# leaner-forever/SEGS-SLAM

Hardware: AMD Instinct MI355X
Metric: mapper train-iters/sec (fwd+bwd raster) (higher is better)
Workload: dtype f32; 1 GPU; 1080p_3m: 3000000 Gaussians, 1920x1080, 1 keyframe per GPU, fwd+bwd raster; P=3000000, P_visible=2096178, num_rendered=10472370, instances_binned=7913347, instances_live=6766534, width=1920, height=1080, parallelism=keyframe-dp1, forward=resident (no host sync), hipgraph=off

## Files before the change

include/segs_raster.h:

```cpp
#ifndef SEGS_RASTER_H_
#define SEGS_RASTER_H_

#include <stddef.h>
#include <stdint.h>

#ifdef __cplusplus
extern "C" {
#endif

#define SEGS_OK 0
#define SEGS_ERR_INVALID_ARGUMENT (-1)
#define SEGS_ERR_UNSUPPORTED (-2)
#define SEGS_ERR_ALLOC (-3)

typedef char* (*segs_alloc_fn)(void* ctx, size_t bytes);

const char* segs_last_error(void);

#define SEGS_RASTER_SKIP_NONPOSITIVE_OPACITY 1u
#define SEGS_RASTER_KEEP_DEAD_INSTANCES 2u
#define SEGS_RASTER_GATHER_TILES_TOUCHED 4u
#define SEGS_RASTER_TEST_NARROW_PACK 8u
#define SEGS_RASTER_UNFUSED_BINNING 16u
#define SEGS_RASTER_TIGHT_BINNING 32u
#define SEGS_RASTER_MFMA_MOMENTS 64u
uint32_t segs_raster_set_flags(uint32_t flags);

uint32_t* segs_raster_set_status_mirror(uint32_t* host_mapped_status);

size_t segs_geometry_bytes(int P);
size_t segs_image_bytes(int width, int height);
size_t segs_binning_bytes(int num_rendered);

int segs_rasterize_forward(segs_alloc_fn geometry_alloc, void* geometry_ctx,
                           segs_alloc_fn binning_alloc, void* binning_ctx,
                           segs_alloc_fn image_alloc, void* image_ctx,
                           int P, int D, int M,
                           const float* background, int width, int height,
                           const float* means3D, const float* shs, const float* colors_precomp,
                           const float* opacities, const float* scales, float scale_modifier,
// ... 28 lines not shown
int segs_project2_image(int P, int D, int M, int width, int height, const float* means3D, const float* shs,
                        const float* colors_precomp, const float* opacities, const float* scales,
                        float scale_modifier, const float* rotations, const float* cov3D_precomp,
                        const float* viewmatrix, const float* projmatrix, const float* cam_pos,
                        float tan_fovx, float tan_fovy, int prefiltered, float* out_color, float* points_image,
                        int* radii, void* stream);

int segs_debug_unpack_geometry(const char* geom_buffer, int P, const int* radii, float* means2D ,
                               float* conic_opacity , float* depths , uint32_t* tiles_touched ,
                               uint32_t* point_offsets , float* rgb , void* stream);
int segs_debug_unpack_binning(const char* binning_buffer, const char* geom_buffer, int P, int R, int width, int height,
                              uint64_t* keys_sorted , uint32_t* point_list , void* stream);
int segs_debug_instance_values(const char* binning_buffer, int R, uint32_t* values , void* stream);
int segs_debug_unpack_image(const char* image_buffer, int width, int height, uint32_t* ranges ,
                            float* final_T , uint32_t* n_contrib , void* stream);

int segs_debug_preprocess_backward(int P, int width, int height, const float* means3D, const int* radii,
                                   const float* scales, float scale_modifier, const float* rotations,
                                   const float* cov3D_precomp, const float* viewmatrix, const float* projmatrix,
                                   float tan_fovx, float tan_fovy, const float* dL_dmean2D, const float* dL_dconic,
                                   float* dL_dmean3D, float* dL_dcov3D, float* dL_dscale, float* dL_drot, void* stream);

int segs_sort_pairs(const uint64_t* keys_in, const uint32_t* vals_in, uint64_t* keys_out, uint32_t* vals_out,
                    int n, int end_bit, char* temp, void* stream);

size_t segs_resident_binning_bytes(int P, int capacity);
int segs_rasterize_forward_resident(char* geom_buffer, char* binning_buffer, char* image_buffer, int capacity,
                                    int geom_rows, int P, int D, int M, const float* background, int width, int height,
                                    const float* means3D, const float* shs, const float* colors_precomp,
                                    const float* opacities, const float* scales, float scale_modifier,
// ... 124 lines not shown
```

segs-slam_amd/_capi.py:

```python
from __future__ import annotations

import ctypes as C
import os
import subprocess

_HERE = os.path.dirname(os.path.abspath(__file__))
CSRC = os.path.join(_HERE, "csrc")
LIB_PATH = os.environ.get("SEGS_RASTER_LIB") or os.path.join(CSRC, "libsegs_raster.so")

ALLOC_FN = C.CFUNCTYPE(C.c_void_p, C.c_void_p, C.c_size_t)


class NeuralDims(C.Structure):
    _fields_ = [("feat_dim", C.c_int), ("n_offsets", C.c_int), ("appearance_dim", C.c_int), ("use_feat_bank", C.c_int),
                ("add_opacity_dist", C.c_int), ("add_cov_dist", C.c_int), ("add_color_dist", C.c_int)]


class ProjectionTargets(C.Structure):
    _fields_ = [("records", C.c_void_p), ("radii", C.c_void_p), ("tiles_touched", C.c_void_p), ("depth_keys", C.c_void_p),
                ("tile_ranges", C.c_void_p), ("depth_overflow", C.c_void_p), ("num_tiles", C.c_int), ("flags", C.c_uint32)]


class DepthOutputs(C.Structure):
    _fields_ = [("depth", C.c_void_p), ("alpha", C.c_void_p)]
# ... 31 lines not shown
    "segs_raster_set_status_mirror": (_vp, [_vp]),
    "segs_training_statis": (_i, [_i, _i] + [_vp] * 9),
    "segs_training_statis_guarded": (_i, [_i, _i] + [_vp] * 10),
    "segs_anchor_growing_temp_bytes": (_sz, [_i, _i]),
    "segs_anchor_growing_level": (_i, [_i, _i, _i, _i] + [_vp] * 7 + [_f, _f, _f, _i] + [_vp] * 5),
    "segs_depth_seed_temp_bytes": (_sz, [_i, _i, _i, _i]),
    "segs_depth_seed": (_i, [_i, _vp, _i, _i, _vp, _vp, _vp, _f, _f, _vp, _vp, _i, _vp, _vp, _vp, _vp, _vp]),
    "segs_neural_set_flags": (C.c_uint, [C.c_uint]),
    "segs_neural_param_layout": (_i, [_vp, _vp, _vp, _vp, _vp]),
    "segs_neural_temp_bytes": (_sz, [_vp, _i]),
    "segs_neural_forward": (_i, [_vp, _i] + [_vp] * 16),
    "segs_neural_forward_projected": (_i, [_vp, _i] + [_vp] * 16 + [_i, _i, _f, _f, _f, _vp, _vp]),
    "segs_neural_backward": (_i, [_vp, _i] + [_vp] * 17 + [_f, _vp, _vp, _vp]),
    "segs_neural_backward_camera": (_i, [_vp, _i] + [_vp] * 17 + [_f, _vp, _vp, _vp, _vp]),
    "segs_geometry_bytes": (_sz, [_i]),
    "segs_image_bytes": (_sz, [_i, _i]),
    "segs_binning_bytes": (_sz, [_i]),
    "segs_rasterize_forward": (_i, [ALLOC_FN, _vp, ALLOC_FN, _vp, ALLOC_FN, _vp, _i, _i, _i, _vp, _i, _i, _vp, _vp, _vp,
                                     _vp, _vp, _f, _vp, _vp, _vp, _vp, _vp, _f, _f, _i, _vp, _vp, _vp, C.POINTER(_i)]),
    "segs_rasterize_backward": (_i, [_i, _i, _i, _i, _vp, _i, _i, _vp, _vp, _vp, _vp, _f, _vp, _vp, _vp, _vp, _vp, _f, _f,
                                      _vp, _vp, _vp, _vp, _vp, _vp, _vp, _vp, _vp, _vp, _vp, _vp, _vp, _vp, _vp]),
    "segs_resident_binning_bytes": (_sz, [_i, _i]),
    "segs_rasterize_forward_resident": (_i, [_vp, _vp, _vp, _i, _i, _i, _i, _i, _vp, _i, _i, _vp, _vp, _vp, _vp, _vp, _f, _vp, _vp, _vp,
                                              _vp, _vp, _f, _f, _vp, _vp, _vp, _vp]),
    "segs_resident_projection_targets": (_i, [_vp, _vp, _vp, _i, _i, _i, _i, _i, _vp, _vp, _vp]),
    "segs_rasterize_forward_resident_projected": (_i, [_vp, _vp, _vp, _i, _i, _i, _vp, _i, _i, _vp, _vp, _vp]),
    "segs_rasterize_backward_resident": (_i, [_vp, _vp, _vp, _i, _i, _i, _i, _i, _vp, _i, _i, _vp, _vp, _vp, _f, _vp, _vp, _vp, _vp, _vp,
                                               _f, _f, _vp, _vp, _vp, _vp, _vp, _vp, _vp, _vp, _vp, _vp, _vp, _vp]),
}
for _name in ("segs_rasterize_forward", "segs_rasterize_backward", "segs_rasterize_forward_resident",
# ... 117 lines not shown
```

segs-slam_amd/csrc/capi.hip:

```cpp
#include <hip/hip_runtime.h>
#include <cstdio>
#include <cstdlib>
#include <algorithm>
#include <cstring>
#include <string>
#include <vector>
#include "../../include/segs_raster.h"
#include "gs_layout.h"
#include "kernels.h"

using namespace segs;

namespace {
thread_local std::string g_err;
}
int segs::set_error(int code, const char* what) {
  g_err = what;
  return code;
}
int segs::set_hip_error(hipError_t e, const char* where) {
  g_err = std::string(where) + ": " + hipGetErrorString(e);
  return (int)e > 0 ? (int)e : 1;
}

// ... 130 lines not shown
  return SEGS_OK;
}

struct Geom {
  GeomLayout L;
  char* base;
  float* rec() const { return (float*)(base + L.rec); }
  BinInfo* bin() const { return (BinInfo*)(base + L.bin); }
  uint32_t* offsets() const { return (uint32_t*)(base + L.offsets); }
  int* radii_internal() const { return (int*)(base + L.radii_internal); }
  uint32_t* block_sums() const { return (uint32_t*)(base + L.block_sums); }
  uint32_t* num_rendered() const { return (uint32_t*)(base + L.num_rendered); }
  uint32_t* clamped() const { return (uint32_t*)(base + L.clamped); }
  float* gacc() const { return (float*)(base + L.gacc); }
  uint32_t* touched() const { return (uint32_t*)(base + L.touched); }
};
Geom geom_at(char* p, int P) { return Geom{geom_layout(P), align_ptr(p)}; }
Geom geom_at(char* p, int P, int rows) {
  Geom g{geom_layout(rows), align_ptr(p)};
  g.L.P = P;
  g.L.nblocks = (P + 255) / 256;
  return g;
}

int run_preprocess(const Geom& G, int P, int W, int H, const float* means3D, const float* colors, const float* opac,
                   const float* scales, float mod, const float* rots, const float* cov3D_precomp, const float* view,
                   const float* proj, float tan_fovx, float tan_fovy, int* radii, const float* shs, int D, int M,
                   const float* cam_pos, hipStream_t st, uint32_t* depth_keys = nullptr, uint32_t* depth_vals = nullptr,
                   uint2* ranges = nullptr, uint32_t extra_flags = 0u, uint32_t* depth_overflow = nullptr) {
  const float focal_y = H / (2.0f * tan_fovy);
// ... 122 lines not shown

uint32_t* segs_raster_set_status_mirror(uint32_t* host_mapped_status) {
  uint32_t* old = g_status_mirror;
  g_status_mirror = host_mapped_status;
  return old;
}

uint32_t segs_raster_set_flags(uint32_t flags) {
  const uint32_t old = g_flags;
  g_flags = flags;
  return old;
}

size_t segs_geometry_bytes(int P) { return geom_layout(P < 0 ? 0 : P).total; }
size_t segs_image_bytes(int width, int height) { return image_layout(width, height).total; }
size_t segs_binning_bytes(int num_rendered) { return binning_layout(num_rendered < 0 ? 0 : num_rendered).total; }

static int rasterize_forward_impl(segs_alloc_fn geometry_alloc, void* geometry_ctx, segs_alloc_fn binning_alloc, void* binning_ctx,
                           segs_alloc_fn image_alloc, void* image_ctx, int P, int D, int M, const float* background,
                           int width, int height, const float* means3D, const float* shs, const float* colors_precomp,
                           const float* opacities, const float* scales, float scale_modifier, const float* rotations,
                           const float* cov3D_precomp, const float* viewmatrix, const float* projmatrix,
                           const float* cam_pos, float tan_fovx, float tan_fovy, int prefiltered, float* out_color,
                           int* radii, const segs_depth_outputs* dout, void* stream, int* num_rendered) {
  (void)prefiltered;
  hipStream_t st = (hipStream_t)stream;
  if (!geometry_alloc || !binning_alloc || !image_alloc) return fail(SEGS_ERR_INVALID_ARGUMENT, "null allocator callback");
  if (P < 0 || width <= 0 || height <= 0) return fail(SEGS_ERR_INVALID_ARGUMENT, "bad P / image size");
  if (P > MAX_GAUSSIANS) return fail(SEGS_ERR_INVALID_ARGUMENT, "P exceeds 2^28 Gaussians (sort values carry a 4-bit quadrant mask)");
  if (!background || !out_color || !viewmatrix || !projmatrix || !num_rendered) return fail(SEGS_ERR_INVALID_ARGUMENT, "null required pointer");
// ... 121 lines not shown
  Geom G = geom_at(geom_buffer, P, geom_rows);
  if (!radii) radii = G.radii_internal();
  const ImageLayout IL = image_layout(width, height);
  const BinningLayout BL = binning_layout(R);
  char* img = align_ptr(image_buffer);
  char* bin = align_ptr(binning_buffer);
  const uint32_t gx = (width + TILE_X - 1) / TILE_X, gy = (height + TILE_Y - 1) / TILE_Y;
  const float focal_y = height / (2.0f * tan_fovy), focal_x = width / (2.0f * tan_fovx);

  if (!self_clean) { PROF(K_MEMSET);
  HIP_TRY(hipMemsetAsync(G.gacc(), 0, (size_t)P * GACC_DWORDS * 4, st));
  }
  const float* dL_ddepth = dgrad ? dgrad->dL_ddepth : nullptr;
  const float* dL_dalpha = dgrad ? dgrad->dL_dalpha : nullptr;
  const bool depth_form = dL_ddepth || dL_dalpha;
  if (R > 0 && depth_form) {
    { PROF(K_RENDER_BWD);
    render_bwd_depth_kernel<<<(gx * gy + 7) / 8 * 32, 64, 0, st>>>((const uint2*)(img + IL.ranges), (const uint32_t*)(bin + BL.vals[0]), width,
                                                                  height, G.rec(), background, (const float*)(img + IL.final_T),
                                                                  (const uint32_t*)(img + IL.n_contrib), dL_dpix, G.gacc(), gx * gy,
                                                                  dL_ddepth, dL_dalpha);
    }
    LAUNCH_TRY("render_bwd_depth_kernel");
  } else if (R > 0) {
    { PROF(K_RENDER_BWD);
    static const bool mfma_env = [] { const char* e = getenv("SEGS_RENDER_BWD_MFMA"); return e && e[0] == '1'; }();
    ((mfma_env || (g_flags & SEGS_RASTER_MFMA_MOMENTS)) ? render_bwd_mfma_kernel : render_bwd_kernel)<<<(gx * gy + 7) / 8 * 32, 64, 0, st>>>((const uint2*)(img + IL.ranges), (const uint32_t*)(bin + BL.vals[0]), width,
                                                    height, G.rec(), background, (const float*)(img + IL.final_T),
                                                    (const uint32_t*)(img + IL.n_contrib), dL_dpix, G.gacc(), gx * gy);
    }
    LAUNCH_TRY("render_bwd_kernel");
  }
  { PROF(K_PREPROCESS_BWD);
  auto* const kernel = cam_live ? (dL_ddepth ? preprocess_bwd_kernel<true, true> : preprocess_bwd_kernel<false, true>)
                                : (dL_ddepth ? preprocess_bwd_kernel<true, false> : preprocess_bwd_kernel<false, false>);
  kernel<<<G.L.nblocks, 256, 0, st>>>(P, means3D, radii, cov3D_precomp ? nullptr : scales, rotations,
                                                     scale_modifier, cov3D_precomp, viewmatrix, projmatrix, focal_x, focal_y,
                                                     tan_fovx, tan_fovy, G.gacc(), (float)width, (float)height, dL_dmean2D, dL_dconic, dL_dopacity, dL_dcolor,
                                                     dL_dmean3D, dL_dcov3D, dL_dscale, dL_drot, self_clean ? 1 : 0, nullptr,
                                                     cam_live ? camera_partials(cam) : nullptr);
  LAUNCH_TRY("preprocess_bwd_kernel");
  if (cam_live)
    if (int rc = camera_grads_finish(cam, G.L.nblocks, st)) return rc;
  }
  if (shs) {
    sh_backward_kernel<<<G.L.nblocks, 256, 0, st>>>(P, means3D, radii, shs, D, M, campos, G.clamped(), dL_dcolor, dL_dmean3D, dL_dsh);
    LAUNCH_TRY("sh_backward_kernel");
  }
  return SEGS_OK;
}

int segs_rasterize_backward(int P, int D, int M, int R, const float* background, int width, int height,
                            const float* means3D, const float* shs, const float* colors_precomp, const float* scales,
                            float scale_modifier, const float* rotations, const float* cov3D_precomp,
                            const float* viewmatrix, const float* projmatrix, const float* campos, float tan_fovx,
// ... 151 lines not shown

int segs_debug_preprocess_backward(int P, int width, int height, const float* means3D, const int* radii, const float* scales,
                                   float scale_modifier, const float* rotations, const float* cov3D_precomp,
                                   const float* viewmatrix, const float* projmatrix, float tan_fovx, float tan_fovy,
                                   const float* dL_dmean2D, const float* dL_dconic, float* dL_dmean3D, float* dL_dcov3D,
                                   float* dL_dscale, float* dL_drot, void* stream) {
  hipStream_t st = (hipStream_t)stream;
  if (P <= 0) return SEGS_OK;
  if (!means3D || !radii || !viewmatrix || !projmatrix || !dL_dmean2D || !dL_dconic || !dL_dmean3D || !dL_dcov3D)
    return fail(SEGS_ERR_INVALID_ARGUMENT, "null pointer");
  const float focal_y = height / (2.0f * tan_fovy), focal_x = width / (2.0f * tan_fovx);
  preprocess_bwd_kernel<false, false><<<(P + 255) / 256, 256, 0, st>>>(P, means3D, radii, cov3D_precomp ? nullptr : scales, rotations,
                                                         scale_modifier, cov3D_precomp, viewmatrix, projmatrix, focal_x, focal_y,
                                                         tan_fovx, tan_fovy, nullptr, (float)width, (float)height, const_cast<float*>(dL_dmean2D),
                                                         const_cast<float*>(dL_dconic), nullptr, nullptr, dL_dmean3D, dL_dcov3D,
                                                         dL_dscale, dL_drot, 0, nullptr, nullptr);
  LAUNCH_TRY("preprocess_bwd_kernel");
  return SEGS_OK;
}

int segs_debug_preprocess_backward_camera(int P, int width, int height, const float* means3D, const int* radii, const float* scales,
                                          float scale_modifier, const float* rotations, const float* cov3D_precomp,
                                          const float* viewmatrix, const float* projmatrix, float tan_fovx, float tan_fovy,
                                          const float* dL_dmean2D, const float* dL_dconic, float* dL_dmean3D, float* dL_dcov3D,
                                          float* dL_dscale, float* dL_drot, const float* dL_dz, const segs_camera_grads* camera_grads,
                                          void* stream) {
  if (!camera_grads)
    return segs_debug_preprocess_backward(P, width, height, means3D, radii, scales, scale_modifier, rotations, cov3D_precomp, viewmatrix,
                                          projmatrix, tan_fovx, tan_fovy, dL_dmean2D, dL_dconic, dL_dmean3D, dL_dcov3D, dL_dscale, dL_drot,
                                          stream);
  hipStream_t st = (hipStream_t)stream;
  bool cam_live = false;
  if (int rc = camera_grads_begin(camera_grads, nullptr, P <= 0, st, &cam_live)) return rc;
  if (P <= 0) return SEGS_OK;
  if (!means3D || !radii || !viewmatrix || !projmatrix || !dL_dmean2D || !dL_dconic || !dL_dmean3D || !dL_dcov3D)
    return fail(SEGS_ERR_INVALID_ARGUMENT, "null pointer");
  const float focal_y = height / (2.0f * tan_fovy), focal_x = width / (2.0f * tan_fovx);
  const int nblocks = (P + 255) / 256;
  (dL_dz ? preprocess_bwd_kernel<true, true> : preprocess_bwd_kernel<false, true>)<<<nblocks, 256, 0, st>>>(
      P, means3D, radii, cov3D_precomp ? nullptr : scales, rotations, scale_modifier, cov3D_precomp, viewmatrix, projmatrix, focal_x,
      focal_y, tan_fovx, tan_fovy, nullptr, (float)width, (float)height, const_cast<float*>(dL_dmean2D), const_cast<float*>(dL_dconic),
      nullptr, nullptr, dL_dmean3D, dL_dcov3D, dL_dscale, dL_drot, 0, dL_dz, camera_partials(camera_grads));
  LAUNCH_TRY("preprocess_bwd_kernel");
  return camera_grads_finish(camera_grads, nblocks, st);
}

int segs_sort_pairs(const uint64_t* keys_in, const uint32_t* vals_in, uint64_t* keys_out, uint32_t* vals_out, int n,
                    int end_bit, char* temp, void* stream) {
  hipStream_t st = (hipStream_t)stream;
  if (n < 0 || end_bit <= 0 || end_bit > 64) return fail(SEGS_ERR_INVALID_ARGUMENT, "bad n / end_bit");
  if (n == 0) return SEGS_OK;
  if (!keys_in || !vals_in || !keys_out || !vals_out || !temp) return fail(SEGS_ERR_INVALID_ARGUMENT, "null pointer");
  const BinningLayout BL = binning_layout(n);
  char* bin = align_ptr(temp);
  const int passes = (end_bit + 7) / 8;
  const int side = passes & 1;
  HIP_TRY(hipMemcpyAsync(bin + BL.keys[side], keys_in, (size_t)n * 8, hipMemcpyDeviceToDevice, st));
// ... 235 lines not shown
```

segs-slam_amd/csrc/gs_layout.h:

```cpp
#pragma once
#include <algorithm>
#include <cstddef>
#include <cstdint>

namespace segs {

constexpr int TILE_X = 16;
constexpr int TILE_Y = 16;
constexpr int NUM_CHANNELS = 3;

constexpr float LOG2E = 1.4426950408889634f;

constexpr int REC_DWORDS = 16;
enum RecField { REC_X = 0, REC_Y, REC_A2, REC_B2, REC_C2, REC_O, REC_R, REC_G, REC_B, REC_DEPTH, REC_RECT_MIN, REC_RECT_MAX, REC_CA, REC_CB, REC_CC };

struct BinInfo { uint32_t depth_bits, rect_min, rect_max, tiles_touched; };
constexpr uint32_t ID_BITS = 28;
constexpr uint32_t ID_MASK = (1u << ID_BITS) - 1u;
constexpr int MAX_GAUSSIANS = 1 << ID_BITS;

constexpr int GACC_DWORDS = 16;

constexpr size_t ALIGN = 256;
inline size_t align_up(size_t v, size_t a = ALIGN) { return (v + a - 1) / a * a; }

struct GeomLayout {
  size_t rec, bin, offsets, radii_internal, block_sums, clamped, num_rendered, gacc, touched, total;
  int P, nblocks;
};
inline GeomLayout geom_layout(int P) {
  GeomLayout g{};
  g.P = P;
  g.nblocks = (P + 255) / 256;
  size_t o = 0;
  g.rec = o;            o = align_up(o + (size_t)P * REC_DWORDS * 4);
  g.bin = o;            o = align_up(o + (size_t)P * sizeof(BinInfo));
  g.offsets = o;        o = align_up(o + (size_t)P * 4);
  g.radii_internal = o; o = align_up(o + (size_t)P * 4);
  g.block_sums = o;     o = align_up(o + (size_t)(g.nblocks + 1) * 4 * 3);
  g.clamped = o;        o = align_up(o + (size_t)P * 4);
  g.num_rendered = o;   o = align_up(o + 64);
  g.gacc = o;           o = align_up(o + (size_t)P * GACC_DWORDS * 4);
  g.touched = o;        o = align_up(o + (size_t)P * 4);
  g.total = o + ALIGN;
  return g;
}

struct ImageLayout {
  size_t ranges, final_T, n_contrib, total;
};
inline ImageLayout image_layout(int W, int H) {
  ImageLayout l{};
  const size_t tiles = (size_t)((W + TILE_X - 1) / TILE_X) * ((H + TILE_Y - 1) / TILE_Y);
  size_t o = 0;
  l.ranges = o;    o = align_up(o + tiles * 8);
  l.final_T = o;   o = align_up(o + (size_t)W * H * 4);
  l.n_contrib = o; o = align_up(o + (size_t)W * H * 4);
  l.total = o + ALIGN;
// ... 58 lines not shown
```

segs-slam_amd/csrc/kernels.h:

```cpp
#pragma once
#include <hip/hip_runtime.h>
#include <cstdint>
#include "gs_layout.h"

namespace segs {

int set_error(int code, const char* what);
int set_hip_error(hipError_t e, const char* where);


__global__ void preprocess_fwd_kernel(
    int P, const float* __restrict__ means3D, const float* __restrict__ scales, float mod,
    const float* __restrict__ rotations, const float* __restrict__ opacities, const float* __restrict__ colors,
    const float* __restrict__ cov3D_precomp, const float* __restrict__ viewmatrix, const float* __restrict__ projmatrix,
    int W, int H, float tan_fovx, float tan_fovy, float focal_x, float focal_y, uint32_t gx, uint32_t gy,
    int* __restrict__ radii, float* __restrict__ rec, BinInfo* __restrict__ bin, uint32_t* __restrict__ block_sums,
    uint32_t* __restrict__ depth_range, const float* __restrict__ shs, int D, int M, const float* __restrict__ cam_pos,
    uint32_t* __restrict__ clamped, uint32_t flags, uint32_t* __restrict__ depth_keys, uint32_t* __restrict__ depth_vals,
    uint2* __restrict__ ranges, int num_tiles, uint32_t* __restrict__ depth_overflow, uint32_t* __restrict__ touched_dense);
constexpr uint32_t DEPTH_KEY_MIN = 0x3E4CCCCDu;
constexpr int DEPTH_KEY_BITS = 27;

__global__ void visible_filter_kernel(
    int P, const float* __restrict__ means3D, const float* __restrict__ scales, float mod,
// ... 3 lines not shown
    int log_scale_stride);

__global__ void mark_visible_kernel(int P, const float* __restrict__ means3D, const float* __restrict__ viewmatrix,
                                    uint8_t* __restrict__ present);

constexpr int CAM_SUMS = 24;
template <bool DEPTH, bool CAM>
__global__ void preprocess_bwd_kernel(
    int P, const float* __restrict__ means3D, const int* __restrict__ radii, const float* __restrict__ scales,
    const float* __restrict__ rotations, float mod, const float* __restrict__ cov3D_precomp,
    const float* __restrict__ view, const float* __restrict__ proj, float h_x, float h_y, float tan_fovx, float tan_fovy,
    float* __restrict__ gacc, float img_w, float img_h,
    float* __restrict__ dL_dmean2D, float* __restrict__ dL_dconic,
    float* __restrict__ dL_dopacity, float* __restrict__ dL_dcolor, float* __restrict__ dL_dmean3D,
    float* __restrict__ dL_dcov3D, float* __restrict__ dL_dscale, float* __restrict__ dL_drot, int clean_gacc,
    const float* __restrict__ dz_in, float* __restrict__ cam_partials);
__global__ void camera_grad_reduce_kernel(const float* __restrict__ partials, int nblocks, float* __restrict__ dL_dview,
                                          float* __restrict__ dL_dproj);
__global__ void sh_backward_kernel(int P, const float* __restrict__ means3D, const int* __restrict__ radii,
                                   const float* __restrict__ shs, int D, int M, const float* __restrict__ cam_pos,
                                   const uint32_t* __restrict__ clamped, const float* __restrict__ dL_dcolor,
                                   float* __restrict__ dL_dmean3D, float* __restrict__ dL_dsh);

__global__ void scan_block_sums_kernel(uint32_t* __restrict__ block_sums, int nblocks, const uint32_t* __restrict__ depth_range,
                                       uint32_t* __restrict__ total);
__global__ void ordered_offsets_kernel(int P, const uint32_t* __restrict__ block_sums, uint32_t* __restrict__ incl,
                                       uint32_t* __restrict__ total_out, const uint32_t* __restrict__ ng_dev,
                                       uint32_t* __restrict__ first_owner, uint32_t owner_entries);
__global__ void duplicate_with_keys_kernel(int P, int R, const float* __restrict__ rec,
                                           const uint32_t* __restrict__ order, const uint32_t* __restrict__ incl,
                                           uint32_t* __restrict__ keys, uint32_t* __restrict__ vals, uint32_t gx,
// ... 15 lines not shown
                                     const uint32_t* __restrict__ digit_totals, int nblocks, int nchunks,
                                     const uint32_t* __restrict__ n_dev, int drop_dead, uint32_t* __restrict__ n_live_out,
                                     const uint32_t* __restrict__ aux_in, uint32_t* __restrict__ aux_out, int nbits, int chunk_tiles, int pack_shift,
                                     uint2* __restrict__ ranges_out, uint32_t* __restrict__ status, uint32_t* __restrict__ status_mirror,
                                     int write_keys);
__global__ void identify_tile_ranges_kernel(int L, const uint32_t* __restrict__ keys, uint2* __restrict__ ranges,
                                            const uint32_t* __restrict__ n_dev, uint32_t* __restrict__ status,
                                            uint32_t* __restrict__ status_mirror, const uint32_t* __restrict__ n_live);

__global__ void render_fwd_kernel(const uint2* __restrict__ ranges, const uint32_t* __restrict__ point_list, int W, int H,
                                  const float* __restrict__ rec, const float* __restrict__ bg,
                                  float* __restrict__ final_T, uint32_t* __restrict__ n_contrib, float* __restrict__ out_color);
__global__ void render_bwd_kernel(const uint2* __restrict__ ranges, const uint32_t* __restrict__ point_list, int W, int H,
                                  const float* __restrict__ rec, const float* __restrict__ bg,
                                  const float* __restrict__ final_T, const uint32_t* __restrict__ n_contrib,
                                  const float* __restrict__ dL_dpix, float* __restrict__ gacc, uint32_t num_tiles);
__global__ void render_bwd_mfma_kernel(const uint2* __restrict__ ranges, const uint32_t* __restrict__ point_list, int W, int H,
                                       const float* __restrict__ rec, const float* __restrict__ bg,
                                       const float* __restrict__ final_T, const uint32_t* __restrict__ n_contrib,
                                       const float* __restrict__ dL_dpix, float* __restrict__ gacc, uint32_t num_tiles);
__global__ void render_fwd_depth_kernel(const uint2* __restrict__ ranges, const uint32_t* __restrict__ point_list, int W, int H,
                                        const float* __restrict__ rec, const float* __restrict__ bg,
                                        float* __restrict__ final_T, uint32_t* __restrict__ n_contrib, float* __restrict__ out_color,
                                        float* __restrict__ out_depth, float* __restrict__ out_alpha);
__global__ void render_bwd_depth_kernel(const uint2* __restrict__ ranges, const uint32_t* __restrict__ point_list, int W, int H,
                                        const float* __restrict__ rec, const float* __restrict__ bg,
                                        const float* __restrict__ final_T, const uint32_t* __restrict__ n_contrib,
                                        const float* __restrict__ dL_dpix, float* __restrict__ gacc, uint32_t num_tiles,
                                        const float* __restrict__ dL_ddepth, const float* __restrict__ dL_dalpha);

__global__ void unpack_geometry_kernel(int P, const float* __restrict__ rec, const BinInfo* __restrict__ bin,
                                       const int* __restrict__ radii, float* __restrict__ means2D,
                                       float* __restrict__ conic_opacity, float* __restrict__ depths,
                                       uint32_t* __restrict__ tiles_touched, float* __restrict__ rgb);

__global__ void rebuild_keys_kernel(int R, const uint32_t* __restrict__ tile_keys, const uint32_t* __restrict__ vals,
                                    const BinInfo* __restrict__ bin, uint64_t* __restrict__ keys64);
__global__ void make_depth_keys_kernel(int P, const BinInfo* __restrict__ bin, uint32_t dcull, uint32_t* __restrict__ keys,
                                       uint32_t* __restrict__ vals, uint2* __restrict__ ranges, int num_tiles);
__global__ void ordered_block_sums_kernel(int P, const uint32_t* touched, const uint32_t* __restrict__ order,
                                          uint32_t* __restrict__ block_sums, uint32_t* sorted_touched,
                                          const uint32_t* __restrict__ ng_dev, uint32_t* __restrict__ order_rw, int pack_shift);
__global__ void point_offsets_kernel(int P, const BinInfo* __restrict__ bin, uint32_t* __restrict__ offsets);
__global__ void strip_mask_kernel(int n, const uint32_t* __restrict__ vals, uint32_t* __restrict__ out);
// ... 3 lines not shown
```

segs-slam_amd/csrc/preprocess.hip:

```cpp
#include <hip/hip_runtime.h>
#include <cstdint>
#include "gs_layout.h"
#include "kernels.h"
#include "project_gaussian.h"
#include "sh_color.h"

#pragma clang fp contract(off)

namespace segs {

__device__ __forceinline__ float3 load_row3(const float* __restrict__ a, int P, float* lds ) {
  const int tid = threadIdx.x;
  const size_t base = (size_t)blockIdx.x * 768;
  const size_t lim = (size_t)P * 3;
#pragma unroll
  for (int k = 0; k < 3; k++) {
    const size_t i = base + k * 256 + tid;
    lds[k * 256 + tid] = i < lim ? a[i] : 0.f;
  }
  __syncthreads();
  float3 v = make_float3(lds[3 * tid], lds[3 * tid + 1], lds[3 * tid + 2]);
  __syncthreads();
  return v;
}
// ... 178 lines not shown
  R[0][0] = 1.f - 2.f * (y * y + z * z); R[0][1] = 2.f * (x * y - r * z);       R[0][2] = 2.f * (x * z + r * y);
  R[1][0] = 2.f * (x * y + r * z);       R[1][1] = 1.f - 2.f * (x * x + z * z); R[1][2] = 2.f * (y * z - r * x);
  R[2][0] = 2.f * (x * z - r * y);       R[2][1] = 2.f * (y * z + r * x);       R[2][2] = 1.f - 2.f * (x * x + y * y);
}

template <bool DEPTH, bool CAM>
__global__ void __launch_bounds__(256) preprocess_bwd_kernel(
    int P, const float* __restrict__ means3D, const int* __restrict__ radii, const float* __restrict__ scales,
    const float* __restrict__ rotations, float mod, const float* __restrict__ cov3D_precomp,
    const float* __restrict__ view, const float* __restrict__ proj, float h_x, float h_y, float tan_fovx, float tan_fovy,
    float* __restrict__ gacc, float img_w, float img_h,
    float* __restrict__ dL_dmean2D, float* __restrict__ dL_dconic,
    float* __restrict__ dL_dopacity, float* __restrict__ dL_dcolor, float* __restrict__ dL_dmean3D,
    float* __restrict__ dL_dcov3D, float* __restrict__ dL_dscale, float* __restrict__ dL_drot,
    int clean_gacc ,
    const float* __restrict__ dz_in, float* __restrict__ cam_partials ) {
  __shared__ float lds[3 * 768];
  const int idx = blockIdx.x * 256 + threadIdx.x;
  const bool live = idx < P;
  const bool binned = live && radii[idx] > 0;
  float3 mean, scale, unused;
  load_rows3(means3D, scales, nullptr, P, lds, mean, scale, unused);

  float g2x = 0.f, g2y = 0.f;
  Sym2 G{0.f, 0.f, 0.f};
  float dcol0 = 0.f, dcol1 = 0.f, dcol2 = 0.f, dop = 0.f, dz = 0.f;
  float4 a0 = make_float4(0.f, 0.f, 0.f, 0.f), a1 = a0;
  if (gacc) {
    {
      __shared__ __attribute__((aligned(16))) float gl[4][32 * GACC_DWORDS];
      const int lane = threadIdx.x & 63;
      float* const wl = gl[threadIdx.x >> 6];
      const uint64_t rows = __ballot(binned);
      const size_t wave_first = (size_t)blockIdx.x * 256 + (threadIdx.x & ~63);
#pragma unroll
      for (int half = 0; half < 2; half++) {
        float4 q[2];
#pragma unroll
        for (int j = 0; j < 2; j++) {
          const int r = 16 * j + (lane >> 2), owner = 32 * half + r;
          q[j] = make_float4(0.f, 0.f, 0.f, 0.f);
          if (((rows >> owner) & 1ull) && (lane & 3) < 3) {
            float4* src = reinterpret_cast<float4*>(gacc + (wave_first + owner) * GACC_DWORDS) + (lane & 3);
            q[j] = *src;
            if (clean_gacc) *src = make_float4(0.f, 0.f, 0.f, 0.f);
          }
        }
#pragma unroll
        for (int j = 0; j < 2; j++) reinterpret_cast<float4*>(wl + (16 * j + (lane >> 2)) * GACC_DWORDS)[lane & 3] = q[j];
// ... 181 lines not shown
    }
  }
  if (gacc) store_row3(dL_dmean2D, P, lds, g2x, g2y, 0.f);
  store_row3(dL_dmean3D, P, lds, out_mean[0], out_mean[1], out_mean[2]);
  if (dL_dscale) store_row3(dL_dscale, P, lds, out_scale[0], out_scale[1], out_scale[2]);
  if (!live) return;
  if (dL_dcov3D) {
#pragma unroll
    for (int e = 0; e < 6; e++) dL_dcov3D[6 * (size_t)idx + e] = out_cov[e];
  }
  if (dL_drot) reinterpret_cast<float4*>(dL_drot)[idx] = make_float4(out_rot[0], out_rot[1], out_rot[2], out_rot[3]);
}

#define SEGS_PREPROCESS_BWD_ARGS int, const float*, const int*, const float*, const float*, float, const float*, const float*, \
    const float*, float, float, float, float, float*, float, float, float*, float*, float*, float*, float*, float*, float*, float*, int, \
    const float*, float*
template __global__ void preprocess_bwd_kernel<false, false>(SEGS_PREPROCESS_BWD_ARGS);
template __global__ void preprocess_bwd_kernel<true, false>(SEGS_PREPROCESS_BWD_ARGS);
template __global__ void preprocess_bwd_kernel<false, true>(SEGS_PREPROCESS_BWD_ARGS);
template __global__ void preprocess_bwd_kernel<true, true>(SEGS_PREPROCESS_BWD_ARGS);
#undef SEGS_PREPROCESS_BWD_ARGS

__global__ void __launch_bounds__(960) camera_grad_reduce_kernel(const float* __restrict__ partials, int nblocks,
                                                                 float* __restrict__ dL_dview, float* __restrict__ dL_dproj) {
  __shared__ float rows[160 * CAM_SUMS];
  __shared__ float mid[10 * CAM_SUMS];
  __shared__ float sums[CAM_SUMS];
  const int t = threadIdx.x, q = t % 6, r0 = t / 6;
  float4 acc = make_float4(0.f, 0.f, 0.f, 0.f);
#pragma unroll 8
  for (int r = r0; r < nblocks; r += 160) {
// ... 39 lines not shown
```

segs-slam_amd/csrc/render.hip:

```cpp
#include <hip/hip_runtime.h>
#include <cstdint>
#include "gs_layout.h"
#include "kernels.h"

namespace segs {

__device__ __forceinline__ uint32_t xcd_tile(uint32_t wg, uint32_t num_tiles) {
  const uint32_t full = num_tiles & ~63u;
  if (wg >= full) return wg;
  const uint32_t xcd = wg & 7u, local = wg >> 3;
  return (local >> 3) * 64u + xcd * 8u + (local & 7u);
}

__device__ __forceinline__ float fast_exp2(float x) { return __builtin_amdgcn_exp2f(x); }
__device__ __forceinline__ float fast_rcp(float x) { return __builtin_amdgcn_rcpf(x); }
__device__ __forceinline__ uint32_t readlane_u32(uint32_t v, int lane) {
  return (uint32_t)__builtin_amdgcn_readlane((int)v, lane);
}


__device__ __forceinline__ float rl(float v, int lane) {
  return __int_as_float(__builtin_amdgcn_readlane(__float_as_int(v), lane));
}

// ... 198 lines not shown
    const float diff = (DEPTH ? (q1.z * dp0 + q1.w * dp1 + q2.x * dp2 + qz * dpz) : (q1.z * dp0 + q1.w * dp1 + q2.x * dp2)) - accd;
    float dL_dalpha = diff * T;
    if (USE_BG) dL_dalpha += (-T_final * rinv) * bg_dot_dpixel;
    accd += ae * diff;
    L.wa[sl][lane] = make_float2(aw * dL_dalpha , ae * T );
  }
}

typedef float f32x4 __attribute__((ext_vector_type(4)));

template <bool MFMA, bool DEPTH>
__device__ __forceinline__ void render_bwd_body(
    const uint2* __restrict__ ranges, const uint32_t* __restrict__ point_list, int W, int H,
    const float* __restrict__ rec, const float* __restrict__ bg, const float* __restrict__ final_T,
    const uint32_t* __restrict__ n_contrib, const float* __restrict__ dL_dpix, float* __restrict__ gacc, uint32_t num_tiles,
    const float* __restrict__ dL_ddepth, const float* __restrict__ dL_dalpha) {
  static_assert(!(MFMA && DEPTH), "the depth form of the tile backward is the VALU form");
  __shared__ BwdLds lds_one;
  const uint32_t tiles_x = (W + TILE_X - 1) / TILE_X;
  const uint32_t xcd = blockIdx.x & 7u, local = blockIdx.x >> 3;
  const uint32_t v = ((local >> 2) << 3) | xcd;
  if (v >= num_tiles) return;
  const uint32_t tile = xcd_tile(v, num_tiles);
  const uint32_t tile_x = tile % tiles_x, tile_y = tile / tiles_x;
  const int lane = threadIdx.x & 63;
  const int wv = __builtin_amdgcn_readfirstlane((int)(local & 3u));
  BwdLds& L = lds_one;
  const uint32_t qx0 = tile_x * TILE_X + (wv & 1) * 8, qy0 = tile_y * TILE_Y + (wv >> 1) * 8;
  const uint32_t px = qx0 + (lane & 7), py = qy0 + (lane >> 3);
  const bool inside = px < (uint32_t)W && py < (uint32_t)H;
  const float pxf = (float)px, pyf = (float)py;
// ... 148 lines not shown
      const float g1 = fold_rows4(S0, S1y, S1x, Sxx);
      const float g2 = fold_rows4(Sxy, Sr, Syy, Sg);
      if (DEPTH) {
        const float g3 = fold_rows4(Sb, Sz, Sb, Sz);
        mom[gs][part] = g1;
        mom[gs][4 + part] = g2;
        if ((part & 1) == 0) mom[gs][8 + (part >> 1)] = g3;
      } else {
      const float g3 = fold_rows4(Sb, Sb, Sb, Sb);
      mom[gs][part] = g1;
      mom[gs][4 + part] = g2;
      if (part == 0) mom[gs][8] = g3;
      }
      }
      wave_lds_fence();
      {
        const float4 m0 = *reinterpret_cast<const float4*>(&mom[gs][0]);
        const float4 m1 = *reinterpret_cast<const float4*>(&mom[gs][4]);
        const float m8 = mom[gs][8];
        const float hx = gxr - cx, hy = gyr - cy;
        const float Mx = hx * m0.x - m0.y, My = hy * m0.x - m0.z;
        const float Mxx = hx * (hx * m0.x - 2.f * m0.y) + m0.w;
        const float Mxy = hx * (hy * m0.x - m0.z) - hy * m0.y + m1.x;
        const float Myy = hy * (hy * m0.x - 2.f * m0.z) + m1.y;
        wave_lds_fence();
        const float inv_o = fast_rcp(reinterpret_cast<const float*>(&L.rec[gs][1])[1]);
        wave_lds_fence();
        if (part == 0) {
          *reinterpret_cast<float4*>(&mom[gs][0]) = make_float4(Mx, My, Mxx, Mxy);
          *reinterpret_cast<float4*>(&mom[gs][4]) = make_float4(Myy, m0.x * inv_o, m1.z, m1.w);
          mom[gs][8] = m8;
        }
      }
      wave_lds_fence();
#pragma unroll
      for (int j = 0; j < 4; j++) {
        const int slot = 4 * j + part;
        if (slot < nb && gs < (DEPTH ? 10 : 9)) {
          const uint32_t id = __float_as_uint(reinterpret_cast<const float*>(&L.rec[slot][2])[2]);
#if !(defined(SEGS_MEASURE) && defined(ABLATE_NO_ATOMICS))
          atomicAdd(gacc + (size_t)id * GACC_DWORDS + gs, mom[slot][gs]);
#endif
        }
      }
      wave_lds_fence();
    } while (taken < n);
    if (tail) break;
  }
}

__global__ void __launch_bounds__(64) render_bwd_kernel(
    const uint2* __restrict__ ranges, const uint32_t* __restrict__ point_list, int W, int H,
    const float* __restrict__ rec, const float* __restrict__ bg, const float* __restrict__ final_T,
    const uint32_t* __restrict__ n_contrib, const float* __restrict__ dL_dpix, float* __restrict__ gacc, uint32_t num_tiles) {
  render_bwd_body<false, false>(ranges, point_list, W, H, rec, bg, final_T, n_contrib, dL_dpix, gacc, num_tiles, nullptr, nullptr);
}
__global__ void __launch_bounds__(64) render_bwd_mfma_kernel(
    const uint2* __restrict__ ranges, const uint32_t* __restrict__ point_list, int W, int H,
    const float* __restrict__ rec, const float* __restrict__ bg, const float* __restrict__ final_T,
    const uint32_t* __restrict__ n_contrib, const float* __restrict__ dL_dpix, float* __restrict__ gacc, uint32_t num_tiles) {
  render_bwd_body<true, false>(ranges, point_list, W, H, rec, bg, final_T, n_contrib, dL_dpix, gacc, num_tiles, nullptr, nullptr);
}
__global__ void __launch_bounds__(64) render_bwd_depth_kernel(
    const uint2* __restrict__ ranges, const uint32_t* __restrict__ point_list, int W, int H,
    const float* __restrict__ rec, const float* __restrict__ bg, const float* __restrict__ final_T,
    const uint32_t* __restrict__ n_contrib, const float* __restrict__ dL_dpix, float* __restrict__ gacc, uint32_t num_tiles,
    const float* __restrict__ dL_ddepth, const float* __restrict__ dL_dalpha) {
  render_bwd_body<false, true>(ranges, point_list, W, H, rec, bg, final_T, n_contrib, dL_dpix, gacc, num_tiles, dL_ddepth, dL_dalpha);
}

}
```

Measured before the change: 980.8 iters/s.

## Track gacc rows written by render backward and skip untouched rows in preprocess backward

Adds a per-Gaussian written byte array to the geometry buffer. Render backward sets the byte for every Gaussian it accumulates into, and preprocess backward treats only those rows as binned. It also limits the gacc clean and zeroes the flags again for the next iteration. This is meant to skip gradient reads, maths and cleanup for Gaussians that were binned but never reached by any pixel, at the cost of extra byte stores in the render backward inner loop and an extra byte read per Gaussian.

Result: faster. 1012 iters/s, median of 6 (+3.2%).

```diff
diff --git a/include/segs_raster.h b/include/segs_raster.h
--- a/include/segs_raster.h
+++ b/include/segs_raster.h
@@ -24,6 +24,7 @@
 #define SEGS_RASTER_UNFUSED_BINNING 16u
 #define SEGS_RASTER_TIGHT_BINNING 32u
 #define SEGS_RASTER_MFMA_MOMENTS 64u
+#define SEGS_RASTER_NO_WRITTEN_BYTES 128u
 uint32_t segs_raster_set_flags(uint32_t flags);
 
 uint32_t* segs_raster_set_status_mirror(uint32_t* host_mapped_status);
@@ -82,6 +83,9 @@
 int segs_debug_instance_values(const char* binning_buffer, int R, uint32_t* values , void* stream);
 int segs_debug_unpack_image(const char* image_buffer, int width, int height, uint32_t* ranges ,
                             float* final_T , uint32_t* n_contrib , void* stream);
+
+#define SEGS_GEOMETRY_REGIONS 10
+int segs_debug_geometry_layout(int P, size_t* offset_and_bytes , int regions);
 
 int segs_debug_preprocess_backward(int P, int width, int height, const float* means3D, const int* radii,
                                    const float* scales, float scale_modifier, const float* rotations,
diff --git a/segs-slam_amd/_capi.py b/segs-slam_amd/_capi.py
--- a/segs-slam_amd/_capi.py
+++ b/segs-slam_amd/_capi.py
@@ -69,6 +69,7 @@
     "segs_neural_backward": (_i, [_vp, _i] + [_vp] * 17 + [_f, _vp, _vp, _vp]),
     "segs_neural_backward_camera": (_i, [_vp, _i] + [_vp] * 17 + [_f, _vp, _vp, _vp, _vp]),
     "segs_geometry_bytes": (_sz, [_i]),
+    "segs_debug_geometry_layout": (_i, [_i, _vp, _i]),
     "segs_image_bytes": (_sz, [_i, _i]),
     "segs_binning_bytes": (_sz, [_i]),
     "segs_rasterize_forward": (_i, [ALLOC_FN, _vp, ALLOC_FN, _vp, ALLOC_FN, _vp, _i, _i, _i, _vp, _i, _i, _vp, _vp, _vp,
diff --git a/segs-slam_amd/csrc/capi.hip b/segs-slam_amd/csrc/capi.hip
--- a/segs-slam_amd/csrc/capi.hip
+++ b/segs-slam_amd/csrc/capi.hip
@@ -168,6 +168,7 @@
   uint32_t* clamped() const { return (uint32_t*)(base + L.clamped); }
   float* gacc() const { return (float*)(base + L.gacc); }
   uint32_t* touched() const { return (uint32_t*)(base + L.touched); }
+  uint8_t* written() const { return (uint8_t*)(base + L.written); }
 };
 Geom geom_at(char* p, int P) { return Geom{geom_layout(P), align_ptr(p)}; }
 Geom geom_at(char* p, int P, int rows) {
@@ -320,6 +321,18 @@
 
 size_t segs_geometry_bytes(int P) { return geom_layout(P < 0 ? 0 : P).total; }
 size_t segs_image_bytes(int width, int height) { return image_layout(width, height).total; }
+
+int segs_debug_geometry_layout(int P, size_t* offset_and_bytes, int regions) {
+  if (P < 0 || !offset_and_bytes || regions != SEGS_GEOMETRY_REGIONS) return fail(SEGS_ERR_INVALID_ARGUMENT, "bad P / region count");
+  const GeomLayout g = geom_layout(P);
+  const size_t p = (size_t)P;
+  const size_t v[SEGS_GEOMETRY_REGIONS][2] = {
+      {g.rec, p * REC_DWORDS * 4}, {g.bin, p * sizeof(BinInfo)}, {g.offsets, p * 4}, {g.radii_internal, p * 4},
+      {g.block_sums, (size_t)(g.nblocks + 1) * 4 * 3}, {g.clamped, p * 4}, {g.num_rendered, 64}, {g.gacc, p * GACC_DWORDS * 4},
+      {g.touched, p * 4}, {g.written, p}};
+  for (int i = 0; i < SEGS_GEOMETRY_REGIONS; i++) { offset_and_bytes[2 * i] = v[i][0]; offset_and_bytes[2 * i + 1] = v[i][1]; }
+  return SEGS_OK;
+}
 size_t segs_binning_bytes(int num_rendered) { return binning_layout(num_rendered < 0 ? 0 : num_rendered).total; }
 
 static int rasterize_forward_impl(segs_alloc_fn geometry_alloc, void* geometry_ctx, segs_alloc_fn binning_alloc, void* binning_ctx,
@@ -471,12 +484,13 @@
   const float* dL_ddepth = dgrad ? dgrad->dL_ddepth : nullptr;
   const float* dL_dalpha = dgrad ? dgrad->dL_dalpha : nullptr;
   const bool depth_form = dL_ddepth || dL_dalpha;
+  uint8_t* const written = (self_clean && !(g_flags & SEGS_RASTER_NO_WRITTEN_BYTES)) ? G.written() : nullptr;
   if (R > 0 && depth_form) {
     { PROF(K_RENDER_BWD);
     render_bwd_depth_kernel<<<(gx * gy + 7) / 8 * 32, 64, 0, st>>>((const uint2*)(img + IL.ranges), (const uint32_t*)(bin + BL.vals[0]), width,
                                                                   height, G.rec(), background, (const float*)(img + IL.final_T),
                                                                   (const uint32_t*)(img + IL.n_contrib), dL_dpix, G.gacc(), gx * gy,
-                                                                  dL_ddepth, dL_dalpha);
+                                                                  dL_ddepth, dL_dalpha, written);
     }
     LAUNCH_TRY("render_bwd_depth_kernel");
   } else if (R > 0) {
@@ -484,7 +498,7 @@
     static const bool mfma_env = [] { const char* e = getenv("SEGS_RENDER_BWD_MFMA"); return e && e[0] == '1'; }();
     ((mfma_env || (g_flags & SEGS_RASTER_MFMA_MOMENTS)) ? render_bwd_mfma_kernel : render_bwd_kernel)<<<(gx * gy + 7) / 8 * 32, 64, 0, st>>>((const uint2*)(img + IL.ranges), (const uint32_t*)(bin + BL.vals[0]), width,
                                                     height, G.rec(), background, (const float*)(img + IL.final_T),
-                                                    (const uint32_t*)(img + IL.n_contrib), dL_dpix, G.gacc(), gx * gy);
+                                                    (const uint32_t*)(img + IL.n_contrib), dL_dpix, G.gacc(), gx * gy, written);
     }
     LAUNCH_TRY("render_bwd_kernel");
   }
@@ -495,7 +509,7 @@
                                                      scale_modifier, cov3D_precomp, viewmatrix, projmatrix, focal_x, focal_y,
                                                      tan_fovx, tan_fovy, G.gacc(), (float)width, (float)height, dL_dmean2D, dL_dconic, dL_dopacity, dL_dcolor,
                                                      dL_dmean3D, dL_dcov3D, dL_dscale, dL_drot, self_clean ? 1 : 0, nullptr,
-                                                     cam_live ? camera_partials(cam) : nullptr);
+                                                     cam_live ? camera_partials(cam) : nullptr, written);
   LAUNCH_TRY("preprocess_bwd_kernel");
   if (cam_live)
     if (int rc = camera_grads_finish(cam, G.L.nblocks, st)) return rc;
@@ -677,7 +691,7 @@
                                                          scale_modifier, cov3D_precomp, viewmatrix, projmatrix, focal_x, focal_y,
                                                          tan_fovx, tan_fovy, nullptr, (float)width, (float)height, const_cast<float*>(dL_dmean2D),
                                                          const_cast<float*>(dL_dconic), nullptr, nullptr, dL_dmean3D, dL_dcov3D,
-                                                         dL_dscale, dL_drot, 0, nullptr, nullptr);
+                                                         dL_dscale, dL_drot, 0, nullptr, nullptr, nullptr);
   LAUNCH_TRY("preprocess_bwd_kernel");
   return SEGS_OK;
 }
@@ -703,7 +717,7 @@
   (dL_dz ? preprocess_bwd_kernel<true, true> : preprocess_bwd_kernel<false, true>)<<<nblocks, 256, 0, st>>>(
       P, means3D, radii, cov3D_precomp ? nullptr : scales, rotations, scale_modifier, cov3D_precomp, viewmatrix, projmatrix, focal_x,
       focal_y, tan_fovx, tan_fovy, nullptr, (float)width, (float)height, const_cast<float*>(dL_dmean2D), const_cast<float*>(dL_dconic),
-      nullptr, nullptr, dL_dmean3D, dL_dcov3D, dL_dscale, dL_drot, 0, dL_dz, camera_partials(camera_grads));
+      nullptr, nullptr, dL_dmean3D, dL_dcov3D, dL_dscale, dL_drot, 0, dL_dz, camera_partials(camera_grads), nullptr);
   LAUNCH_TRY("preprocess_bwd_kernel");
   return camera_grads_finish(camera_grads, nblocks, st);
 }
diff --git a/segs-slam_amd/csrc/gs_layout.h b/segs-slam_amd/csrc/gs_layout.h
--- a/segs-slam_amd/csrc/gs_layout.h
+++ b/segs-slam_amd/csrc/gs_layout.h
@@ -25,7 +25,7 @@
 inline size_t align_up(size_t v, size_t a = ALIGN) { return (v + a - 1) / a * a; }
 
 struct GeomLayout {
-  size_t rec, bin, offsets, radii_internal, block_sums, clamped, num_rendered, gacc, touched, total;
+  size_t rec, bin, offsets, radii_internal, block_sums, clamped, num_rendered, gacc, touched, written, total;
   int P, nblocks;
 };
 inline GeomLayout geom_layout(int P) {
@@ -42,6 +42,7 @@
   g.num_rendered = o;   o = align_up(o + 64);
   g.gacc = o;           o = align_up(o + (size_t)P * GACC_DWORDS * 4);
   g.touched = o;        o = align_up(o + (size_t)P * 4);
+  g.written = o;        o = align_up(o + (size_t)P);
   g.total = o + ALIGN;
   return g;
 }
diff --git a/segs-slam_amd/csrc/kernels.h b/segs-slam_amd/csrc/kernels.h
--- a/segs-slam_amd/csrc/kernels.h
+++ b/segs-slam_amd/csrc/kernels.h
@@ -41,7 +41,7 @@
     float* __restrict__ dL_dmean2D, float* __restrict__ dL_dconic,
     float* __restrict__ dL_dopacity, float* __restrict__ dL_dcolor, float* __restrict__ dL_dmean3D,
     float* __restrict__ dL_dcov3D, float* __restrict__ dL_dscale, float* __restrict__ dL_drot, int clean_gacc,
-    const float* __restrict__ dz_in, float* __restrict__ cam_partials);
+    const float* __restrict__ dz_in, float* __restrict__ cam_partials, uint8_t* __restrict__ written);
 __global__ void camera_grad_reduce_kernel(const float* __restrict__ partials, int nblocks, float* __restrict__ dL_dview,
                                           float* __restrict__ dL_dproj);
 __global__ void sh_backward_kernel(int P, const float* __restrict__ means3D, const int* __restrict__ radii,
@@ -87,11 +87,13 @@
 __global__ void render_bwd_kernel(const uint2* __restrict__ ranges, const uint32_t* __restrict__ point_list, int W, int H,
                                   const float* __restrict__ rec, const float* __restrict__ bg,
                                   const float* __restrict__ final_T, const uint32_t* __restrict__ n_contrib,
-                                  const float* __restrict__ dL_dpix, float* __restrict__ gacc, uint32_t num_tiles);
+                                  const float* __restrict__ dL_dpix, float* __restrict__ gacc, uint32_t num_tiles,
+                                  uint8_t* __restrict__ written);
 __global__ void render_bwd_mfma_kernel(const uint2* __restrict__ ranges, const uint32_t* __restrict__ point_list, int W, int H,
                                        const float* __restrict__ rec, const float* __restrict__ bg,
                                        const float* __restrict__ final_T, const uint32_t* __restrict__ n_contrib,
-                                       const float* __restrict__ dL_dpix, float* __restrict__ gacc, uint32_t num_tiles);
+                                       const float* __restrict__ dL_dpix, float* __restrict__ gacc, uint32_t num_tiles,
+                                       uint8_t* __restrict__ written);
 __global__ void render_fwd_depth_kernel(const uint2* __restrict__ ranges, const uint32_t* __restrict__ point_list, int W, int H,
                                         const float* __restrict__ rec, const float* __restrict__ bg,
                                         float* __restrict__ final_T, uint32_t* __restrict__ n_contrib, float* __restrict__ out_color,
@@ -100,7 +102,8 @@
                                         const float* __restrict__ rec, const float* __restrict__ bg,
                                         const float* __restrict__ final_T, const uint32_t* __restrict__ n_contrib,
                                         const float* __restrict__ dL_dpix, float* __restrict__ gacc, uint32_t num_tiles,
-                                        const float* __restrict__ dL_ddepth, const float* __restrict__ dL_dalpha);
+                                        const float* __restrict__ dL_ddepth, const float* __restrict__ dL_dalpha,
+                                        uint8_t* __restrict__ written);
 
 __global__ void unpack_geometry_kernel(int P, const float* __restrict__ rec, const BinInfo* __restrict__ bin,
                                        const int* __restrict__ radii, float* __restrict__ means2D,
diff --git a/segs-slam_amd/csrc/preprocess.hip b/segs-slam_amd/csrc/preprocess.hip
--- a/segs-slam_amd/csrc/preprocess.hip
+++ b/segs-slam_amd/csrc/preprocess.hip
@@ -216,11 +216,13 @@
     float* __restrict__ dL_dopacity, float* __restrict__ dL_dcolor, float* __restrict__ dL_dmean3D,
     float* __restrict__ dL_dcov3D, float* __restrict__ dL_dscale, float* __restrict__ dL_drot,
     int clean_gacc ,
-    const float* __restrict__ dz_in, float* __restrict__ cam_partials ) {
+    const float* __restrict__ dz_in, float* __restrict__ cam_partials ,
+    uint8_t* __restrict__ written) {
   __shared__ float lds[3 * 768];
   const int idx = blockIdx.x * 256 + threadIdx.x;
   const bool live = idx < P;
-  const bool binned = live && radii[idx] > 0;
+  const bool row_written = (gacc && written) ? (live && written[idx] != 0) : live;
+  const bool binned = live && radii[idx] > 0 && row_written;
   float3 mean, scale, unused;
   load_rows3(means3D, scales, nullptr, P, lds, mean, scale, unused);
 
@@ -233,8 +235,10 @@
       __shared__ __attribute__((aligned(16))) float gl[4][32 * GACC_DWORDS];
       const int lane = threadIdx.x & 63;
       float* const wl = gl[threadIdx.x >> 6];
-      const uint64_t rows = __ballot(binned);
+      const uint64_t rows = __ballot(written ? row_written : binned);
       const size_t wave_first = (size_t)blockIdx.x * 256 + (threadIdx.x & ~63);
+      if (written && clean_gacc && rows != 0ull && lane < 16 && wave_first + 4 * lane < (size_t)P)
+        reinterpret_cast<uint32_t*>(written + wave_first)[lane] = 0u;
 #pragma unroll
       for (int half = 0; half < 2; half++) {
         float4 q[2];
@@ -446,7 +450,7 @@
 
 #define SEGS_PREPROCESS_BWD_ARGS int, const float*, const int*, const float*, const float*, float, const float*, const float*, \
     const float*, float, float, float, float, float*, float, float, float*, float*, float*, float*, float*, float*, float*, float*, int, \
-    const float*, float*
+    const float*, float*, uint8_t*
 template __global__ void preprocess_bwd_kernel<false, false>(SEGS_PREPROCESS_BWD_ARGS);
 template __global__ void preprocess_bwd_kernel<true, false>(SEGS_PREPROCESS_BWD_ARGS);
 template __global__ void preprocess_bwd_kernel<false, true>(SEGS_PREPROCESS_BWD_ARGS);
diff --git a/segs-slam_amd/csrc/render.hip b/segs-slam_amd/csrc/render.hip
--- a/segs-slam_amd/csrc/render.hip
+++ b/segs-slam_amd/csrc/render.hip
@@ -236,7 +236,7 @@
     const uint2* __restrict__ ranges, const uint32_t* __restrict__ point_list, int W, int H,
     const float* __restrict__ rec, const float* __restrict__ bg, const float* __restrict__ final_T,
     const uint32_t* __restrict__ n_contrib, const float* __restrict__ dL_dpix, float* __restrict__ gacc, uint32_t num_tiles,
-    const float* __restrict__ dL_ddepth, const float* __restrict__ dL_dalpha) {
+    const float* __restrict__ dL_ddepth, const float* __restrict__ dL_dalpha, uint8_t* __restrict__ written) {
   static_assert(!(MFMA && DEPTH), "the depth form of the tile backward is the VALU form");
   __shared__ BwdLds lds_one;
   const uint32_t tiles_x = (W + TILE_X - 1) / TILE_X;
@@ -415,6 +415,7 @@
       }
       }
       wave_lds_fence();
+      uint32_t id_gs;
       {
         const float4 m0 = *reinterpret_cast<const float4*>(&mom[gs][0]);
         const float4 m1 = *reinterpret_cast<const float4*>(&mom[gs][4]);
@@ -426,6 +427,7 @@
         const float Myy = hy * (hy * m0.x - 2.f * m0.z) + m1.y;
         wave_lds_fence();
         const float inv_o = fast_rcp(reinterpret_cast<const float*>(&L.rec[gs][1])[1]);
+        id_gs = __float_as_uint(reinterpret_cast<const float*>(&L.rec[gs][2])[2]);
         wave_lds_fence();
         if (part == 0) {
           *reinterpret_cast<float4*>(&mom[gs][0]) = make_float4(Mx, My, Mxx, Mxy);
@@ -444,6 +446,11 @@
 #endif
         }
       }
+      if (written && lane < nb) {
+        uint32_t one;
+        asm volatile("v_mov_b32 %0, 1" : "=v"(one));
+        written[id_gs] = (uint8_t)one;
+      }
       wave_lds_fence();
     } while (taken < n);
     if (tail) break;
@@ -453,21 +460,23 @@
 __global__ void __launch_bounds__(64) render_bwd_kernel(
     const uint2* __restrict__ ranges, const uint32_t* __restrict__ point_list, int W, int H,
     const float* __restrict__ rec, const float* __restrict__ bg, const float* __restrict__ final_T,
-    const uint32_t* __restrict__ n_contrib, const float* __restrict__ dL_dpix, float* __restrict__ gacc, uint32_t num_tiles) {
-  render_bwd_body<false, false>(ranges, point_list, W, H, rec, bg, final_T, n_contrib, dL_dpix, gacc, num_tiles, nullptr, nullptr);
+    const uint32_t* __restrict__ n_contrib, const float* __restrict__ dL_dpix, float* __restrict__ gacc, uint32_t num_tiles,
+    uint8_t* __restrict__ written) {
+  render_bwd_body<false, false>(ranges, point_list, W, H, rec, bg, final_T, n_contrib, dL_dpix, gacc, num_tiles, nullptr, nullptr, written);
 }
 __global__ void __launch_bounds__(64) render_bwd_mfma_kernel(
-    const uint2* __restrict__ ranges, const uint32_t* __restrict__ point_list, int W, int H,
-    const float* __restrict__ rec, const float* __restrict__ bg, const float* __restrict__ final_T,
-    const uint32_t* __restrict__ n_contrib, const float* __restrict__ dL_dpix, float* __restrict__ gacc, uint32_t num_tiles) {
-  render_bwd_body<true, false>(ranges, point_list, W, H, rec, bg, final_T, n_contrib, dL_dpix, gacc, num_tiles, nullptr, nullptr);
-}
-__global__ void __launch_bounds__(64) render_bwd_depth_kernel(
     const uint2* __restrict__ ranges, const uint32_t* __restrict__ point_list, int W, int H,
     const float* __restrict__ rec, const float* __restrict__ bg, const float* __restrict__ final_T,
     const uint32_t* __restrict__ n_contrib, const float* __restrict__ dL_dpix, float* __restrict__ gacc, uint32_t num_tiles,
-    const float* __restrict__ dL_ddepth, const float* __restrict__ dL_dalpha) {
-  render_bwd_body<false, true>(ranges, point_list, W, H, rec, bg, final_T, n_contrib, dL_dpix, gacc, num_tiles, dL_ddepth, dL_dalpha);
-}
-
-}
+    uint8_t* __restrict__ written) {
+  render_bwd_body<true, false>(ranges, point_list, W, H, rec, bg, final_T, n_contrib, dL_dpix, gacc, num_tiles, nullptr, nullptr, written);
+}
+__global__ void __launch_bounds__(64) render_bwd_depth_kernel(
+    const uint2* __restrict__ ranges, const uint32_t* __restrict__ point_list, int W, int H,
+    const float* __restrict__ rec, const float* __restrict__ bg, const float* __restrict__ final_T,
+    const uint32_t* __restrict__ n_contrib, const float* __restrict__ dL_dpix, float* __restrict__ gacc, uint32_t num_tiles,
+    const float* __restrict__ dL_ddepth, const float* __restrict__ dL_dalpha, uint8_t* __restrict__ written) {
+  render_bwd_body<false, true>(ranges, point_list, W, H, rec, bg, final_T, n_contrib, dL_dpix, gacc, num_tiles, dL_ddepth, dL_dalpha, written);
+}
+
+}
```
